# HKUST-Aerial-Robotics/A-LOAM

Hardware: AMD Instinct MI355X
Metric: HDL-64 scans/sec (whole node) (higher is better)
Workload: dtype f32 features / f64 solve

## Files before the change

a-loam_amd/csrc/aloam_capi.hip:

```cpp
#include <algorithm>
#include <cstdio>
#include <cstdlib>
#include <cstring>

#include "capi_internal.hpp"
#include "information_device.hpp"

namespace aloam {

hipEvent_t prof_event(aloam_ctx* c) {
  if (!c->prof_free.empty()) { hipEvent_t e = c->prof_free.back(); c->prof_free.pop_back(); return e; }
  Event e;
  (void)hipEventCreate(&e.h);
  c->prof_events.push_back(std::move(e));
  return c->prof_events.back();
}

int stage_ints(aloam_ctx* c, const int* src, int n, int* dst) {
  const int ns = c->h_nin_slot;
  c->h_nin_slot = (ns + 1) % kNinSlots;
  int* slot = c->h_nin.get() + (size_t)ns * c->B;
  if (c->nin_used[ns]) HIP_TRY(c, hipEventSynchronize(c->nin_done[ns]));
  std::memcpy(slot, src, sizeof(int) * n);
  HIP_TRY(c, hipMemcpyAsync(dst, slot, sizeof(int) * n, hipMemcpyHostToDevice, c->stream));
// ... 112 lines not shown
  { int cus = 0; if (hipDeviceGetAttribute(&cus, hipDeviceAttributeMultiprocessorCount, cfg->device) == hipSuccess && cus > 0) c->gather_blocks = 8 * cus; }
  if (reg) {
    c->slab = c->npad + 16;
    if ((rc = dmalloc(c, c->d_slabs, B * R * (size_t)c->slab))) return rc;
    if ((rc = dmalloc(c, c->d_front_lb, B * NB * (size_t)kFrontSlots))) return rc;
    if ((rc = dmalloc(c, c->d_front_ticket, B))) return rc;
    if ((rc = dmalloc(c, c->d_ringstart, B * (R + 1)))) return rc;
    if ((rc = dmalloc(c, c->d_curv, B * cap))) return rc;
    if ((rc = dmalloc(c, c->d_label, B * cap))) return rc;
    if ((rc = dmalloc(c, c->d_lookback, B * 4 * R))) return rc;
    if ((rc = dmalloc(c, c->d_ring_ticket, B))) return rc;
  }
  if (reg || odo) {
    if ((rc = dmalloc(c, c->d_sharp, B * R * kSharpPerRing))) return rc;
    if ((rc = dmalloc(c, c->d_flat, B * R * kFlatPerRing))) return rc;
  }
  for (int k = 0; k < 2; ++k) {
    if (!(odo || (k == 0 && reg) || (k == 1 && map))) continue;
    if ((rc = dmalloc(c, c->d_less_sharp[k], B * R * kLessSharpPerRing))) return rc;
    if ((rc = dmalloc(c, c->d_less_flat[k], B * cap))) return rc;
  }
  if (odo) {
    for (int p = 0; p < 2; ++p) for (int k = 0; k < 2; ++k) {
      const size_t per = k == 0 ? R * kLessSharpPerRing : cap;
      if ((rc = dmalloc(c, c->d_grid_sorted3[p][k], B * per))) return rc;
      if ((rc = dmalloc(c, c->d_grid_sorted2[p][k], B * per))) return rc;
      if ((rc = dmalloc(c, c->d_grid_start3[p][k], B * (c->grid_H[k] + 1)))) return rc;
      if ((rc = dmalloc(c, c->d_grid_start2[p][k], B * (c->grid_H[k] + 1)))) return rc;
      if ((rc = dmalloc(c, c->d_grid_sorted3c[p][k], B * per))) return rc;
      if ((rc = dmalloc(c, c->d_grid_start3c[p][k], B * (c->grid_H[k] + 1)))) return rc;
      if ((rc = dmalloc(c, c->d_grid_flags[p][k], B * 4))) return rc;
      if ((rc = dmalloc(c, c->d_grid_walk[p][k], B * 2 * (R + 8)))) return rc;
    }
    if (c->grid_overlap) {
      HIP_TRY(c, hipStreamCreateWithFlags(&c->grid_stream.h, hipStreamNonBlocking));
      HIP_TRY(c, hipEventCreateWithFlags(&c->grid_fork.h, hipEventDisableTiming));
      HIP_TRY(c, hipEventCreateWithFlags(&c->grids_done.h, hipEventDisableTiming));
    }
    if ((rc = dmalloc(c, c->d_edges, B * R * kSharpPerRing))) return rc;
    if ((rc = dmalloc(c, c->d_planes, B * R * kFlatPerRing))) return rc;
    if ((rc = dmalloc(c, c->d_sel_sharp, B * R * kSharpPerRing))) return rc;
    if ((rc = dmalloc(c, c->d_sel_flat, B * R * kFlatPerRing))) return rc;
    if ((rc = prepare_build_grids(c->grid_H[1]))) { c->err = "k_build_grids: dynamic LDS size rejected"; return ALOAM_E_HIP; }
  }
  std::vector<OdomState> init(B);
  std::memset(init.data(), 0, sizeof(OdomState) * B);
  for (size_t b = 0; b < B; ++b) { init[b].para_q[3] = 1.0; init[b].q_w[3] = 1.0; }
  HIP_TRY(c, hipMemcpyAsync(c->d_state.get(), init.data(), sizeof(OdomState) * B, hipMemcpyHostToDevice, c->stream));
  HIP_TRY(c, hipStreamSynchronize(c->stream));
  return ALOAM_OK;
}

void aloam_destroy(aloam_ctx* c) {
  DeviceScope device_scope(c);
  if (!c) return;
  if (c->stream) (void)hipStreamSynchronize(c->stream);
  if (c->copy_stream) (void)hipStreamSynchronize(c->copy_stream);
  if (c->grid_stream) (void)hipStreamSynchronize(c->grid_stream);
  prof_resolve(c);
  delete c;
}

const char* aloam_last_error(const aloam_ctx* c) { return c ? c->err.c_str() : "null context"; }
void* aloam_stream(aloam_ctx* c) { return c ? (void*)c->stream : nullptr; }

int aloam_synchronize(aloam_ctx* c) {
  DeviceScope device_scope(c);
// ... 162 lines not shown
```

a-loam_amd/csrc/aloam_device.hpp:

```cpp
#pragma once
#include <hip/hip_runtime.h>
#include <stdint.h>
#include "aloam_atan.hpp"

namespace aloam {

constexpr int kFrontSlots = 128 + 8;
constexpr int kBlockPts = 1024;
constexpr int kMaxRings = 128;
constexpr int kSectors = 6;
constexpr int kSharpPerSector = 2;
constexpr int kLessSharpPerSector = 20;
constexpr int kFlatPerSector = 4;
constexpr int kSharpPerRing = kSectors * kSharpPerSector;
constexpr int kLessSharpPerRing = kSectors * kLessSharpPerSector;
constexpr int kFlatPerRing = kSectors * kFlatPerSector;
constexpr int kNnTile = 1024;

enum ErrBits { kErrEmpty = 1, kErrRingCap = 2, kErrPointCap = 4, kErrInternal = 8 };

struct alignas(16) SeqMeta {
  int n_in;
  int first_kept, last_kept;
  int half_idx;
// ... 31 lines not shown
  int pt_stride;
  int B, cap, R, NB;
  int ring_from_field;
  float min_range;
  SeqMeta* meta;
  float4* slabs;
  int slab;
  unsigned long long* front_lb;
  int* front_ticket;
  int* ringstart;
  float4* cloud;
  float* curv;
  int8_t* label;
  unsigned long long* lookback;
  unsigned epoch;
  int* ring_ticket;
  int store_debug;
  float4* sharp;
  float4* less_sharp[2];
  float4* flat;
  float4* less_flat[2];
  const int* active;
};

constexpr int kRangeRowTables = 6;
struct RangeArgs {
  const int* n_cols;
  const float2* az_xy;
  const float* row_tab;
  int rows, n_az, row_major;
  float range_scale;
};

struct OdomArgs {
  int B, cap, R;
  SeqMeta* meta;
  OdomState* state;
  const float4* sharp;
  const float4* flat;
  const float4* less_sharp[2];
  const float4* less_flat[2];
  const int* active;
  float4* grid_sorted3[2][2];
  float4* grid_sorted2[2][2];
  int* grid_start3[2][2];
  int* grid_start2[2][2];
  float4* grid_sorted3c[2][2];
  int* grid_start3c[2][2];
  int* grid_flags[2][2];
  int* grid_walk[2][2];
  int grid_H_corner, grid_H_surf;
  float4* sel_sharp;
  float4* sel_flat;
  EdgeRec* edges;
  PlaneRec* planes;
  int outer;
  int last_outer;
  int lm_max_iterations;
  int distortion;
};

template <typename T>
__device__ __forceinline__ T* row_of(T* const (&buf)[2], int k, int b, long long per) { return (k ? buf[1] : buf[0]) + b * per; }
__device__ __forceinline__ const float4* corner_last(const OdomArgs& a, int b, int parity) { return row_of(a.less_sharp, parity ^ 1, b, (long long)a.R * kLessSharpPerRing); }
__device__ __forceinline__ const float4* surf_last(const OdomArgs& a, int b, int parity) { return row_of(a.less_flat, parity ^ 1, b, (long long)a.cap); }

struct GridView {
  int H;
  float4 *sorted3, *sorted2, *sorted3c;
  int *start3, *start2, *start3c, *flags, *walk;
};
template <typename T>
__device__ __forceinline__ T* grid_ptr(T* const (&buf)[2][2], int set, int which) {
  return set ? (which ? buf[1][1] : buf[1][0]) : (which ? buf[0][1] : buf[0][0]);
}
__device__ __forceinline__ GridView grid_view(const OdomArgs& a, int b, int which, int set) {
  GridView g;
  g.H = which == 0 ? a.grid_H_corner : a.grid_H_surf;
  const long long per = which == 0 ? (long long)a.R * kLessSharpPerRing : (long long)a.cap;
  g.sorted3 = grid_ptr(a.grid_sorted3, set, which) + b * per;
  g.sorted2 = grid_ptr(a.grid_sorted2, set, which) + b * per;
  g.start3 = grid_ptr(a.grid_start3, set, which) + (long long)b * (g.H + 1);
  g.start2 = grid_ptr(a.grid_start2, set, which) + (long long)b * (g.H + 1);
  g.sorted3c = grid_ptr(a.grid_sorted3c, set, which) + b * per;
// ... 185 lines not shown
```

a-loam_amd/csrc/capi_internal.hpp:

```cpp
#pragma once
#include <hip/hip_runtime.h>

#include <cstdio>
#include <memory>
#include <string>
#include <utility>
#include <vector>

#include "../../include/aloam_mi355x.h"
#include "aloam_device.hpp"
#include "atlas_kernels.hpp"
#include "checkpoint_kernels.hpp"
#include "export_kernels.hpp"
#include "mapping_kernels.hpp"
#include "odometry_kernels.hpp"
#include "places_kernels.hpp"
#include "posegraph_kernels.hpp"
#include "registration_kernels.hpp"
#include "relocalize_kernels.hpp"

using namespace aloam;

namespace aloam {
enum KernelId { K_FIND_ENDS = 0, K_FRONT, K_RING_STARTS, K_DENSE_CLOUD, K_RING_FEATURES, K_BUILD_GRIDS, K_TRANSFORM, K_ASSOC_CORNER,
// ... 71 lines not shown
  aloam_config cfg{};
  int stages = ALOAM_STAGE_ALL;
  int B = 0, cap = 0, R = 0, NB = 0, npad = 0;
  int max_points = 0;
  std::string err;
  DevBuf<char> d_in[2]; size_t d_in_bytes[2] = {0, 0};
  int in_slot = 0;
  bool in_used[2] = {false, false};
  DevBuf<int> d_nin;
  PinnedBuf<int> h_nin; int h_nin_slot = 0;
  bool nin_used[kNinSlots] = {};
  std::vector<SeqHost> seq;
  bool all_active = true, any_frozen = false, any_attached = false;
  bool reg_pending = false;
  const int* reg_mask = nullptr;
  DevBuf<int> d_mask_reg, d_mask_odo, d_mask_map, d_reset_ids;
  DevBuf<SeqMeta> d_meta;
  DevBuf<float4> d_slabs; int slab = 0;
  DevBuf<unsigned long long> d_front_lb; DevBuf<int> d_front_ticket;
  bool dense_valid = true;
  DevBuf<int> d_ringstart;
  DevBuf<float4> d_cloud; DevBuf<float> d_curv; DevBuf<int8_t> d_label;
  DevBuf<unsigned long long> d_lookback; unsigned reg_epoch = 0;
  DevBuf<int> d_ring_ticket;
  bool debug_arrays = false;
  DevBuf<float4> d_sharp, d_flat;
  DevBuf<float4> d_less_sharp[2], d_less_flat[2];
  DevBuf<OdomState> d_state;
  DevBuf<float4> d_grid_sorted3[2][2], d_grid_sorted2[2][2];
  DevBuf<int> d_grid_start3[2][2], d_grid_start2[2][2];
  DevBuf<float4> d_grid_sorted3c[2][2];
  DevBuf<int> d_grid_start3c[2][2];
  DevBuf<int> d_grid_flags[2][2], d_grid_walk[2][2];
  int grid_H[2] = {4096, 16384};
  bool grid_overlap = false;
  DevBuf<EdgeRec> d_edges; DevBuf<PlaneRec> d_planes;
  DevBuf<float4> d_sel_sharp, d_sel_flat;
  bool map_on = false;
  long long map_err_reported = 0;
  float map_line_res = 0.4f, map_plane_res = 0.8f;
  int map_levels = 0, map_stack_tile_bound = 0, map_nsegs_max = 0;
  MapPool map;
  int map_pool_limit = 1 << 26;
  int map_growths = 0;
  long long map_steps = 0;
  int nin_max = 0;
  int inject_max = 0;
  PinnedBuf<volatile int> h_map_report;
  int* d_map_report_host = nullptr;
  DevBuf<int> d_map_report, d_map_live;
  DevBuf<MapSeq> d_mapseq; DevBuf<CubeDesc> d_cubes; DevBuf<int> d_maptab;
  DevBuf<MapGridSig> d_grid_sig;
  DevBuf<float4> d_stack[2], d_stack_world[2]; DevBuf<int> d_stack_cube[2];
  DevBuf<int> d_addcnt, d_cursor, d_compact_flag;
  DevBuf<MapEdgeRec> d_medges; DevBuf<MapNormRec> d_mnorms; DevBuf<float4> d_registered, d_knn;
  DevBuf<int> d_vox_lists;
  DevBuf<int> d_rec_tiles; int rec_tiles_corner = 0, rec_tiles_per_seq = 0;
  DevBuf<VoxSeg> d_segs; DevBuf<int> d_vox_counters, d_bbox;
  DevBuf<int> d_exp_cnt, d_exp_chunk; DevBuf<long long> d_exp_off;
  DevBuf<int> d_exp_pref[2];
  int exp_last_segs = 0;
  int gather_blocks = 2048;
  DevBuf<float4> d_exp_tmp; long long exp_tmp_cap = 0;
  DevBuf<long long> d_exp_tmp_off;
  DevBuf<int> d_ck_seqs, d_ck_info, d_ck_units, d_ck_chunk, d_ck_pref; DevBuf<long long> d_ck_uoff;
  PinnedBuf<char> h_ck; char* d_ck_host = nullptr;
// ... 183 lines not shown
```

a-loam_amd/csrc/capi_odometry.hip:

```cpp
#include <algorithm>
#include <cstring>

#include "capi_internal.hpp"

namespace {

RegArgs reg_args(aloam_ctx* c, const void* d_scans, long long seq_stride, int pt_stride) {
  RegArgs a{};
  a.in = (const char*)d_scans; a.seq_stride = seq_stride; a.pt_stride = pt_stride;
  a.B = c->B; a.cap = c->cap; a.R = c->R; a.NB = c->NB;
  a.ring_from_field = c->cfg.ring_from_field; a.min_range = c->cfg.min_range;
  a.meta = c->d_meta.get(); a.slabs = c->d_slabs.get(); a.slab = c->slab; a.front_lb = c->d_front_lb.get(); a.front_ticket = c->d_front_ticket.get();
  a.ringstart = c->d_ringstart.get(); a.cloud = c->d_cloud.get(); a.curv = c->d_curv.get(); a.label = c->d_label.get();
  a.lookback = c->d_lookback.get(); a.epoch = c->reg_epoch; a.store_debug = c->debug_arrays ? 1 : 0; a.ring_ticket = c->d_ring_ticket.get();
  a.sharp = c->d_sharp.get(); a.flat = c->d_flat.get();
  for (int k = 0; k < 2; ++k) { a.less_sharp[k] = c->d_less_sharp[k].get(); a.less_flat[k] = c->d_less_flat[k].get(); }
  a.active = c->reg_mask;
  return a;
}

}

namespace aloam {

OdomArgs odom_args(aloam_ctx* c) {
  OdomArgs a{};
  a.B = c->B; a.cap = c->cap; a.R = c->R;
  a.meta = c->d_meta.get(); a.state = c->d_state.get();
  a.sharp = c->d_sharp.get(); a.flat = c->d_flat.get();
  for (int k = 0; k < 2; ++k) { a.less_sharp[k] = c->d_less_sharp[k].get(); a.less_flat[k] = c->d_less_flat[k].get(); }
  for (int p = 0; p < 2; ++p) for (int k = 0; k < 2; ++k) {
    a.grid_sorted3[p][k] = c->d_grid_sorted3[p][k].get(); a.grid_sorted2[p][k] = c->d_grid_sorted2[p][k].get(); a.grid_start3[p][k] = c->d_grid_start3[p][k].get();
    a.grid_sorted3c[p][k] = c->d_grid_sorted3c[p][k].get(); a.grid_start3c[p][k] = c->d_grid_start3c[p][k].get();
    a.grid_start2[p][k] = c->d_grid_start2[p][k].get();
    a.grid_flags[p][k] = c->d_grid_flags[p][k].get(); a.grid_walk[p][k] = c->d_grid_walk[p][k].get();
  }
  a.grid_H_corner = c->grid_H[0]; a.grid_H_surf = c->grid_H[1];
  a.edges = c->d_edges.get(); a.planes = c->d_planes.get();
  a.sel_sharp = c->d_sel_sharp.get(); a.sel_flat = c->d_sel_flat.get();
  a.lm_max_iterations = c->cfg.lm_max_iterations;
  a.distortion = c->cfg.distortion != 0;
  return a;
}

}

namespace {

int check_batch(aloam_ctx* c, const int* n_in, int stride_bytes) {
  if (const int rc = require_stage(c, ALOAM_STAGE_REGISTRATION)) return rc;
  if (stride_bytes < 12 || (stride_bytes & 3)) { c->err = "stride_bytes must be 12 (x, y, z only) or >= 16, and a multiple of 4"; return ALOAM_E_ARG; }
  if (stride_bytes == 12 && c->cfg.ring_from_field) { c->err = "ring_from_field needs the 4th float of every record: stride_bytes >= 16"; return ALOAM_E_ARG; }
  for (int b = 0; b < c->B; ++b) {
    if (n_in[b] < 0) { c->err = "negative point count"; return ALOAM_E_ARG; }
    if (n_in[b] > c->max_points) { c->err = "scan exceeds max_points"; return ALOAM_E_CAPACITY; }
  }
  return ALOAM_OK;
}

}

namespace aloam {

int register_launch(aloam_ctx* c, const void* d_scans, long long seq_stride, const int* n_in, int stride_bytes, int slot, bool debug_arrays, const int* n_cols) {
  int rc = ALOAM_OK;
  if (!c->all_active && (rc = ensure_dense(c))) return rc;
  c->nin_max = 0;
  for (int b = 0; b < c->B; ++b) if (takes_part(c, b)) c->nin_max = std::max(c->nin_max, n_in[b]);
  if ((rc = stage_ints(c, n_cols ? n_cols : n_in, c->B, c->d_nin.get()))) return rc;
  if (n_cols) c->range_cols.assign(n_cols, n_cols + c->B); else c->range_cols.clear();
// ... 143 lines not shown
  const int rc = stage_and_register(c, h_scans, seq_stride_bytes, n_in, stride_bytes, false);
  if (rc) return rc;
  return aloam_odometry_step(c);
}

int aloam_input_consumed(aloam_ctx* c) {
  DeviceScope device_scope(c);
  if (!c) return ALOAM_E_ARG;
  for (int s = 0; s < 2; ++s) if (c->in_used[s]) HIP_TRY(c, hipEventSynchronize(c->in_consumed[s]));
  return ALOAM_OK;
}

int aloam_odometry_step(aloam_ctx* c) {
  DeviceScope device_scope(c);
  if (!c) return ALOAM_E_ARG;
  if (const int rc = require_stage(c, ALOAM_STAGE_ODOMETRY)) return rc;
  if (!c->have_features) { c->err = "aloam_odometry_step before any features were registered / set"; return ALOAM_E_STATE; }
  StageMask m;
  if (const int rc = stage_mask(c, c->d_mask_odo, [](const SeqHost& s) { return s.inited ? (int)kSeqSolve : 0; },
                                [](const aloam_ctx* x, const StageMask& k) { return k.all_solve || (!k.any_solve && x->all_active); }, &m)) return rc;
  const int* mask = m.dev;
  const bool any_solve = m.any_solve;
  const bool overlap = c->grid_overlap;
  bool build_last = !overlap;
  if (overlap) for (int b = 0; b < c->B; ++b) build_last |= (m.bits[b] & kSeqSolve) && !c->seq[b].grid_built;
  hipError_t join_err = hipSuccess;
  const int cus = c->gather_blocks / 8;
  auto launch_all = [&]() {
    OdomArgs a = odom_args(c);
    a.active = mask;
    if (overlap) {
      hipError_t e = hipEventRecord(c->grid_fork, c->stream);
      if (e == hipSuccess) e = hipStreamWaitEvent(c->grid_stream, c->grid_fork, 0);
      { ProfScope p(c, K_BUILD_GRIDS, c->grid_stream); launch_build_grids(a, true, cus, c->grid_stream); }
      if (e == hipSuccess) e = hipEventRecord(c->grids_done, c->grid_stream);
      join_err = e;
    }
    if (any_solve && build_last) {
      if (overlap) launch_build_grids(a, false, cus, c->stream);
      else { ProfScope p(c, K_BUILD_GRIDS); launch_build_grids(a, false, cus, c->stream); }
    }
    for (int outer = 0; any_solve && outer < c->cfg.outer_iterations; ++outer) {
      a.outer = outer;
      a.last_outer = outer == c->cfg.outer_iterations - 1;
      { ProfScope p(c, K_TRANSFORM); launch_transform_queries(a, c->stream); }
      { ProfScope p(c, K_ASSOC_CORNER); launch_associate(a, false, c->stream); }
      { ProfScope p(c, K_ASSOC_PLANE); launch_associate(a, true, c->stream); }
      { ProfScope p(c, K_SOLVE); launch_solve(a, c->stream); }
    }
    if (overlap && join_err == hipSuccess) join_err = hipStreamWaitEvent(c->stream, c->grids_done, 0);
    { ProfScope p(c, K_ADVANCE); launch_advance(a, c->stream); }
  };
  if (!any_solve) {
    launch_all();
  } else if (c->use_graph && !c->prof_on && !c->debug_sync) {
    GraphExec& ge = c->odom_graph[mask ? 1 : 0];
    if (!ge) {
      hipGraph_t g = nullptr;
      hipError_t e = hipStreamBeginCapture(c->stream, hipStreamCaptureModeThreadLocal);
      if (e == hipSuccess) {
        launch_all();
        e = hipStreamEndCapture(c->stream, &g);
        if (e == hipSuccess) e = hipGraphInstantiate(&ge.h, g, nullptr, nullptr, 0);
        if (g) (void)hipGraphDestroy(g);
      }
      if (e != hipSuccess) {
        (void)hipGetLastError();
        ge.reset();
        c->use_graph = false;
      }
    }
    if (ge) HIP_TRY(c, hipGraphLaunch(ge, c->stream));
    else launch_all();
// ... 214 lines not shown
```

a-loam_amd/csrc/odometry_kernels.hip:

```cpp
#include "aloam_device.hpp"
#include "aloam_trig.hpp"
#include "lm_device.hpp"
#include "odometry_solve_device.hpp"
#include "odometry_kernels.hpp"

namespace aloam {

#define ALOAM_PHASE(name) asm volatile("; ##PHASE " name)
#ifdef ALOAM_PHASE_CLOCK
__device__ unsigned long long g_phase_clock_odo[2][32];
#define ALOAM_BG_CLOCK(slot) do { if (threadIdx.x == 0 && blockIdx.x == 1) { atomicAdd(&g_phase_clock_odo[0][slot], (unsigned long long)__builtin_readcyclecounter()); atomicAdd(&g_phase_clock_odo[1][slot], 1ull); } } while (0)
#else
#define ALOAM_BG_CLOCK(slot) do { } while (0)
#endif
#ifdef ALOAM_ASSOC_STATS
__device__ unsigned long long g_assoc_stats[2][32];
#define ALOAM_STAT(cls, i, v) do { if ((threadIdx.x & 63) == 0) atomicAdd(&g_assoc_stats[cls][i], (unsigned long long)(v)); } while (0)
#else
#define ALOAM_STAT(cls, i, v) do { } while (0)
#endif

__device__ __forceinline__ float4 transform_to_start(const float4& p, const OdomState& st) {
  double q[4] = {st.para_q[0], st.para_q[1], st.para_q[2], st.para_q[3]};
  if (q[3] < 0.0) { q[0] = -q[0]; q[1] = -q[1]; q[2] = -q[2]; q[3] = -q[3]; }
// ... 25 lines not shown
    const int i = base + tid;
    const int key = i < n ? (int)pts[i].w : -1;
    const int prev = __shfl_up(key, 1, 64), next = __shfl_down(key, 1, 64);
    if (key >= 0 && key < S) {
      if (lane == 0 || prev != key) atomicMin(&s_first[key], i);
      if (lane == 63 || next != key) atomicMax(&s_last[key], i);
    }
  }
  __syncthreads();
  if (tid == 0) {
    int run = n;
    for (int k = S - 1; k >= 0; --k) { run = min(run, s_first[k]); s_first[k] = run; walk[k] = run; }
    run = -1;
    for (int k = 0; k < S; ++k) { run = max(run, s_last[k]); s_last[k] = run; walk[S + k] = run; }
    bool nearly = true;
    for (int k = 3; k < S; ++k) nearly = nearly && s_last[k - 3] < s_first[k];
    s_flag[1] = nearly ? 1 : 2;
  }
  __syncthreads();
}
__host__ __device__ __forceinline__ bool fused_takes(int n, int H) { return n <= kFusedMaxN && H <= kFusedMaxH; }

template <bool NEXT>
struct BuildSrc {
  int n, set;
  const float4* pts;
  __device__ __forceinline__ BuildSrc(const OdomArgs& a, const SeqMeta& m, int b, int which) {
    set = NEXT ? m.parity : m.parity ^ 1;
    n = which == 0 ? (NEXT ? m.n_less_sharp : m.n_corner_last) : (NEXT ? m.n_less_flat : m.n_surf_last);
    pts = which == 0 ? row_of(a.less_sharp, set, b, (long long)a.R * kLessSharpPerRing) : row_of(a.less_flat, set, b, (long long)a.cap);
  }
};

template <bool NEXT>
__device__ __forceinline__ void build_grids_fused(const OdomArgs& a, int b, int which) {
  constexpr int U = 4;
  const int tid = threadIdx.x, lane = tid & 63, wave = tid >> 6;
  if (seq_idle(a.active, b, NEXT ? kSeqActive : kSeqSolve)) return;
  const SeqMeta m = a.meta[b];
  const BuildSrc<NEXT> src(a, m, b, which);
  const int n = src.n;
  const float4* pts = src.pts;
  const GridView g = grid_view(a, b, which, src.set);
  const int H = g.H;
  if (!fused_takes(n, H)) return;
  extern __shared__ __attribute__((aligned(16))) int lds[];
  unsigned* tab = reinterpret_cast<unsigned*>(lds);
  int* s_part = lds + 3 * (H / 2);
  int* s_flag = s_part + 48;
  int* s_walk = s_flag + 8;
  int* const starts[3] = {g.start3, g.start3c, g.start2};
  if (n == 0) {
    for (int t = 0; t < 3; ++t) for (int h = tid; h <= H; h += 1024) starts[t][h] = 0;
    if (tid < 3) g.flags[tid] = 0;
    return;
  }
  ALOAM_BG_CLOCK(0);
  for (int w = tid; w < 3 * (H / 2); w += 1024) tab[w] = 0u;
  if (tid < 2) s_flag[tid] = 0;
  __syncthreads();
  ALOAM_BG_CLOCK(1);
  const float inv0 = 1.0f / cell3_of(which), inv1 = 1.0f / (cell3_of(which) * kCell3CoarseFactor), inv2 = 1.0f / kCell2;
  const unsigned hm = (unsigned)(H - 1);
  auto buckets = [&](const float4& p, int key, unsigned* h) {
    h[0] = hash3((int)floorf(p.x * inv0), (int)floorf(p.y * inv0), (int)floorf(p.z * inv0)) & hm;
    h[1] = hash3((int)floorf(p.x * inv1), (int)floorf(p.y * inv1), (int)floorf(p.z * inv1)) & hm;
    h[2] = hash3((int)floorf(p.x * inv2), (int)floorf(p.y * inv2), key) & hm;
  };
  auto fetch = [&](int base, float4* p) {
#pragma unroll
    for (int u = 0; u < U; ++u) { const int i = base + u * 1024 + tid; p[u] = pts[i < n ? i : n - 1]; }
  };
  {
    int bad = 0, unsorted = 0;
    for (int base = 0; base < n; base += U * 1024) {
      float4 p[U];
      float pw[U];
      fetch(base, p);
// ... 47 lines not shown
    }
  }
  __syncthreads();
  ALOAM_BG_CLOCK(4);
  for (int base = 0; base < n; base += U * 1024) {
    float4 p[U];
    fetch(base, p);
#pragma unroll
    for (int u = 0; u < U; ++u) {
      const int i = base + u * 1024 + tid;
      if (i >= n) continue;
      const int key = (int)p[u].w;
      unsigned h[3];
      buckets(p[u], key, h);
      unsigned pos[3];
#pragma unroll
      for (int t = 0; t < 3; ++t) {
        const unsigned sh = (h[t] & 1u) * 16;
        pos[t] = (atomicAdd(&tab[t * (H / 2) + (h[t] >> 1)], 1u << sh) >> sh) & 0xffffu;
      }
      const float4 e = make_float4(p[u].x, p[u].y, p[u].z, __uint_as_float((unsigned)i | ((unsigned)(key + 1) << 20)));
      g.sorted3[pos[0]] = e;
      g.sorted3c[pos[1]] = e;
      g.sorted2[pos[2]] = e;
    }
  }
  ALOAM_BG_CLOCK(5);
#ifdef ALOAM_PHASE_CLOCK
  __syncthreads();
  ALOAM_BG_CLOCK(6);
#endif
}

__global__ __launch_bounds__(1024) void k_build_grids_fused(OdomArgs a) { build_grids_fused<false>(a, blockIdx.y, blockIdx.x); }
__global__ __launch_bounds__(1024) void k_build_grids_fused_next(OdomArgs a) {
  const int G = gridDim.x;
  for (int r = 0, i = blockIdx.x; i < 2 * a.B; ++r, i += G) {
    build_grids_fused<true>(a, i >> 1, (i ^ r) & 1);
    __syncthreads();
  }
}

constexpr int kBgWaves = 4;
constexpr int kBgUnroll = 4;
template <bool NEXT>
__device__ __forceinline__ void build_grids(const OdomArgs& a) {
  constexpr int U = kBgUnroll;
  const int b = blockIdx.y, which = blockIdx.x / 3, tid = threadIdx.x;
  const int pass_lo = blockIdx.x % 3, pass_hi = pass_lo + 1;
  if (seq_idle(a.active, b, NEXT ? kSeqActive : kSeqSolve)) return;
  const SeqMeta m = a.meta[b];
  const BuildSrc<NEXT> src(a, m, b, which);
  const int n = src.n;
  const float4* pts = src.pts;
  const GridView g = grid_view(a, b, which, src.set);
  if (fused_takes(n, g.H)) return;
  extern __shared__ __attribute__((aligned(16))) int lds[];
  int* cnt = lds;
  int* part = lds + g.H;
  int* s_flag = part + 1024;
  if (tid < 2) s_flag[tid] = n >= (1 << 20) && tid == 0 ? 1 : 0;
  if (n == 0) {
    for (int pass = pass_lo; pass < pass_hi; ++pass) { int* st = pass == 0 ? g.start3 : pass == 1 ? g.start3c : g.start2; for (int h = tid; h <= g.H; h += 1024) st[h] = 0; }
    if (tid < 3 && pass_lo == 0) g.flags[tid] = 0;
    return;
  }
  auto fetch = [&](int base, float4* p) {
#pragma unroll
    for (int u = 0; u < U; ++u) { const int i = base + u * 1024 + tid; p[u] = pts[i < n ? i : n - 1]; }
  };
  for (int pass = pass_lo; pass < pass_hi; ++pass) {
    const bool g3 = pass < 2;
    const float cell = pass == 0 ? cell3_of(which) : pass == 1 ? cell3_of(which) * kCell3CoarseFactor : kCell2;
    const float inv = 1.0f / cell;
    int* start = pass == 0 ? g.start3 : pass == 1 ? g.start3c : g.start2;
    float4* sorted = pass == 0 ? g.sorted3 : pass == 1 ? g.sorted3c : g.sorted2;
    __syncthreads();
    for (int h = tid; h < g.H; h += 1024) cnt[h] = 0;
    __syncthreads();
    float4 p[U], pn[U];
    float pw[U], pwn[U];
    fetch(0, p);
    if (pass == 0) {
#pragma unroll
      for (int u = 0; u < U; ++u) { const int i = u * 1024 + tid; pw[u] = pts[i < n ? (i > 0 ? i - 1 : 0) : n - 1].w; }
    }
    int bad = 0, unsorted = 0;
    for (int base = 0; base < n; base += U * 1024) {
      if (base + U * 1024 < n) {
// ... 21 lines not shown
    if (pass == 0) {
      if (bad) atomicOr(&s_flag[0], 1);
      if (unsorted) atomicOr(&s_flag[1], 1);
    }
    __syncthreads();
    if (pass == 0 && tid < 3) g.flags[tid] = tid == 2 ? 0 : (tid == 1 ? 2 * s_flag[1] : s_flag[0]);
    const int per = g.H / 1024;
    int local = 0;
    for (int k = 0; k < per; ++k) local += cnt[tid * per + k];
    int total;
    int run = block_exclusive_scan<int, 1024>(local, part, &total);
    for (int k = 0; k < per; ++k) { const int c = cnt[tid * per + k]; cnt[tid * per + k] = run; start[tid * per + k] = run; run += c; }
    if (tid == 1023) start[g.H] = run;
    __syncthreads();
    fetch(0, p);
    for (int base = 0; base < n; base += U * 1024) {
      if (base + U * 1024 < n) fetch(base + U * 1024, pn);
#pragma unroll
      for (int u = 0; u < U; ++u) {
        const int i = base + u * 1024 + tid;
        if (i >= n) continue;
        const int key = (int)p[u].w;
        const int ix = (int)floorf(p[u].x * inv), iy = (int)floorf(p[u].y * inv);
        const int iz = g3 ? (int)floorf(p[u].z * inv) : key;
        const int pos = atomicAdd(&cnt[hash3(ix, iy, iz) & (g.H - 1)], 1);
        sorted[pos] = make_float4(p[u].x, p[u].y, p[u].z, __uint_as_float((unsigned)i | ((unsigned)(key + 1) << 20)));
      }
#pragma unroll
      for (int u = 0; u < U; ++u) p[u] = pn[u];
    }
  }
}

__global__ __launch_bounds__(1024, kBgWaves) void k_build_grids(OdomArgs a) { build_grids<false>(a); }
__global__ __launch_bounds__(1024, kBgWaves) void k_build_grids_next(OdomArgs a) { build_grids<true>(a); }

__device__ __forceinline__ float walk_dist(const float4& p, const float4& sel) {
  return (p.x - sel.x) * (p.x - sel.x) + (p.y - sel.y) * (p.y - sel.y) + (p.z - sel.z) * (p.z - sel.z);
}

__device__ __forceinline__ unsigned long long wave_min_u64(unsigned long long v) {
  return wave_min_packed(v);
}

__device__ __forceinline__ void ring2d(int r, int t, int* dx, int* dy) {
  const int w = 2 * r + 1;
  if (t < w) { *dx = -r + t; *dy = -r; }
  else if (t < 2 * w) { *dx = -r + (t - w); *dy = r; }
  else { const int u = t - 2 * w, side = u / (w - 2); *dy = -r + 1 + u % (w - 2); *dx = side ? r : -r; }
}
__device__ __forceinline__ void shell3d(int r, int c, int* dx, int* dy, int* dz) {
  const int w = 2 * r + 1, nface = w * w;
  if (c < 2 * nface) { const int f = c / nface, q = c % nface; *dz = f ? r : -r; *dy = q / w - r; *dx = q % w - r; }
  else { const int q = c - 2 * nface; *dz = -r + 1 + q / (8 * r); ring2d(r, q % (8 * r), dx, dy); }
}

template <int kSweep> struct Kept { float4 p[kSweep]; bool a[kSweep]; bool ok; };

template <int kSweep, class F>
__device__ __forceinline__ void wave_sweep(const float4* __restrict__ sorted, int s0, int cnt, int lane, int* row, F&& f, Kept<kSweep>* keep = nullptr) {
  const int incl = wave_scan_i32<false>(cnt);
  const int total = __builtin_amdgcn_readlane(incl, 63);
  const int excl = incl - cnt;
  int carry = 0;
  for (int base = 0; base < total; base += kSweep * 64) {
    const int slot = excl - base;
    const int rows = total - base > (kSweep - 1) * 64 ? kSweep : (total - base + 63) >> 6;
#pragma unroll
// ... 769 lines not shown
    st.lm_iterations[o] = iterations;
    st.lm_successful[o] = successful;
    st.initial_cost[o] = initial_cost;
    st.final_cost[o] = cost;
    st.termination[o] = termination;
    if (a.last_outer) {
      const double qw[4] = {st.q_w[0], st.q_w[1], st.q_w[2], st.q_w[3]};
      double rt[3];
      quat_rotate(qw, t[0], t[1], t[2], rt);
      st.t_w[0] += rt[0]; st.t_w[1] += rt[1]; st.t_w[2] += rt[2];
      st.q_w[0] = qw[3] * q[0] + qw[0] * q[3] + qw[1] * q[2] - qw[2] * q[1];
      st.q_w[1] = qw[3] * q[1] + qw[1] * q[3] + qw[2] * q[0] - qw[0] * q[2];
      st.q_w[2] = qw[3] * q[2] + qw[2] * q[3] + qw[0] * q[1] - qw[1] * q[0];
      st.q_w[3] = qw[3] * q[3] - qw[0] * q[0] - qw[1] * q[1] - qw[2] * q[2];
    }
  }
}

__global__ void k_advance(SeqMeta* meta, OdomState* state, const int* active, int B) {
  const int b = blockIdx.x * blockDim.x + threadIdx.x;
  if (b >= B || seq_idle(active, b)) return;
  SeqMeta& m = meta[b];
  m.n_corner_last = m.n_less_sharp; m.n_surf_last = m.n_less_flat; m.parity ^= 1;
  state[b].inited = 1;
}
__global__ void k_set_inited(OdomState* state, int B, int inited) {
  const int b = blockIdx.x * blockDim.x + threadIdx.x;
  if (b < B) state[b].inited = inited;
}
void launch_set_inited(OdomState* state, int B, int inited, hipStream_t s) { hipLaunchKernelGGL(k_set_inited, dim3((B + 63) / 64), dim3(64), 0, s, state, B, inited); }
void launch_advance(const OdomArgs& a, hipStream_t s) { hipLaunchKernelGGL(k_advance, dim3((a.B + 63) / 64), dim3(64), 0, s, a.meta, a.state, a.active, a.B); }

size_t build_grids_lds_bytes(int H, int R) { return sizeof(int) * ((size_t)H + 1024 + 2 * (R + 8) + 4); }
static size_t build_grids_fused_lds_bytes(int H) { return sizeof(int) * (3 * (size_t)(H / 2) + 48 + 8 + 2 * kWalkKeys); }
int prepare_build_grids(int H_surf) {
  const int fused = (int)build_grids_fused_lds_bytes(kFusedMaxH), per_grid = (int)build_grids_lds_bytes(H_surf, kMaxRings);
  if (hipFuncSetAttribute((const void*)k_build_grids_fused, hipFuncAttributeMaxDynamicSharedMemorySize, fused) != hipSuccess) return -1;
  if (hipFuncSetAttribute((const void*)k_build_grids_fused_next, hipFuncAttributeMaxDynamicSharedMemorySize, fused) != hipSuccess) return -1;
  if (hipFuncSetAttribute((const void*)k_build_grids, hipFuncAttributeMaxDynamicSharedMemorySize, per_grid) != hipSuccess) return -1;
  return hipFuncSetAttribute((const void*)k_build_grids_next, hipFuncAttributeMaxDynamicSharedMemorySize, per_grid) == hipSuccess ? 0 : -1;
}
void launch_build_grids(const OdomArgs& a, bool next, int cus, hipStream_t s) {
  const int hc = a.grid_H_corner <= kFusedMaxH ? a.grid_H_corner : 0, hs = a.grid_H_surf <= kFusedMaxH ? a.grid_H_surf : 0;
  const size_t fused = build_grids_fused_lds_bytes(hc > hs ? hc : hs), per_grid = build_grids_lds_bytes(a.grid_H_surf, a.R);
  if (next) {
    const int wgs = cus / 2 >= 2 ? (cus / 2) & ~1 : 2;
    if (hc || hs) hipLaunchKernelGGL(k_build_grids_fused_next, dim3(2 * a.B < wgs ? 2 * a.B : wgs), dim3(1024), fused, s, a);
    hipLaunchKernelGGL(k_build_grids_next, dim3(6, a.B), dim3(1024), per_grid, s, a);
  } else {
    if (hc || hs) hipLaunchKernelGGL(k_build_grids_fused, dim3(2, a.B), dim3(1024), fused, s, a);
    hipLaunchKernelGGL(k_build_grids, dim3(6, a.B), dim3(1024), per_grid, s, a);
  }
}
void launch_transform_queries(const OdomArgs& a, hipStream_t s) {
  const dim3 grid((a.R * (kSharpPerRing + kFlatPerRing) + 255) / 256, a.B);
  if (a.distortion) hipLaunchKernelGGL(k_transform_queries<true>, grid, dim3(256), 0, s, a);
  else hipLaunchKernelGGL(k_transform_queries<false>, grid, dim3(256), 0, s, a);
}
void launch_associate(const OdomArgs& a, bool plane, hipStream_t s) {
  const int by = (a.B + 7) / 8 * 8;
  const int qcap = plane ? a.R * kFlatPerRing : a.R * kSharpPerRing;
  const bool wide = a.R > 64;
  const dim3 grid((unsigned)(qcap / 2 * by)), block(64), gridf((unsigned)a.B), blockf(256);
  const dim3 gridn((unsigned)((qcap / 2 + kPairsPerWave - 1) / kPairsPerWave), (unsigned)a.B);
  if (wide) {
    if (plane) { hipLaunchKernelGGL((k_associate_pair<true, true>), grid, block, 0, s, a); hipLaunchKernelGGL((k_associate_nearly<true, true>), gridn, block, 0, s, a); hipLaunchKernelGGL((k_associate_flagged<true, true>), gridf, blockf, 0, s, a); }
    else { hipLaunchKernelGGL((k_associate_pair<false, true>), grid, block, 0, s, a); hipLaunchKernelGGL((k_associate_nearly<false, true>), gridn, block, 0, s, a); hipLaunchKernelGGL((k_associate_flagged<false, true>), gridf, blockf, 0, s, a); }
  } else {
    if (plane) { hipLaunchKernelGGL((k_associate_pair<true, false>), grid, block, 0, s, a); hipLaunchKernelGGL((k_associate_nearly<true, false>), gridn, block, 0, s, a); hipLaunchKernelGGL((k_associate_flagged<true, false>), gridf, blockf, 0, s, a); }
    else { hipLaunchKernelGGL((k_associate_pair<false, false>), grid, block, 0, s, a); hipLaunchKernelGGL((k_associate_nearly<false, false>), gridn, block, 0, s, a); hipLaunchKernelGGL((k_associate_flagged<false, false>), gridf, blockf, 0, s, a); }
  }
}
void launch_solve(const OdomArgs& a, hipStream_t s) {
  if (a.distortion) hipLaunchKernelGGL(k_solve<true>, dim3(a.B), dim3(kSolveThreads), 0, s, a);
  else hipLaunchKernelGGL(k_solve<false>, dim3(a.B), dim3(kSolveThreads), 0, s, a);
}
}

#ifdef ALOAM_PHASE_CLOCK
extern "C" int aloam_debug_phase_clock_odo(unsigned long long* out) { return (int)hipMemcpyFromSymbol(out, HIP_SYMBOL(aloam::g_phase_clock_odo), sizeof(unsigned long long) * 64); }
#endif
#ifdef ALOAM_ASSOC_STATS
extern "C" int aloam_debug_assoc_stats(unsigned long long* out) { return (int)hipMemcpyFromSymbol(out, HIP_SYMBOL(aloam::g_assoc_stats), sizeof(unsigned long long) * 64); }
#endif
// ... 1 lines not shown
```

a-loam_amd/csrc/odometry_kernels.hpp:

```cpp
#pragma once
#include "aloam_device.hpp"

struct aloam_pose_information;

namespace aloam {
size_t build_grids_lds_bytes(int H, int R);
int prepare_build_grids(int H_surf);
void launch_build_grids(const OdomArgs& a, bool next, int cus, hipStream_t s);
void launch_transform_queries(const OdomArgs& a, hipStream_t s);
void launch_associate(const OdomArgs& a, bool plane, hipStream_t s);
void launch_solve(const OdomArgs& a, hipStream_t s);
void launch_advance(const OdomArgs& a, hipStream_t s);
void launch_pose_information_odom(const OdomArgs& a, const int* list, int n, aloam_pose_information* dst, hipStream_t s);
void launch_set_inited(OdomState* state, int B, int inited, hipStream_t s);
}
```

Measured before the change: 134,700.

## Build non-fused grids from a device work list with persistent workgroups

Fused grid builds that decline a cloud now append its three pass items to a device work list. The per-grid kernel then runs as a persistent grid sized to resident capacity and pulls items from that list with an atomic counter, replacing a 6xB launch where most blocks exited early. It also adds register caps and a kernarg reload trick to cut register pressure, plus an env knob to split the corner and surface fused launches. Risks include atomic contention, correctness of the list reset by the last block, and spills under the forced register limits.

```diff
diff --git a/a-loam_amd/csrc/aloam_capi.hip b/a-loam_amd/csrc/aloam_capi.hip
--- a/a-loam_amd/csrc/aloam_capi.hip
+++ b/a-loam_amd/csrc/aloam_capi.hip
@@ -168,7 +168,16 @@
       if ((rc = dmalloc(c, c->d_grid_flags[p][k], B * 4))) return rc;
       if ((rc = dmalloc(c, c->d_grid_walk[p][k], B * 2 * (R + 8)))) return rc;
     }
+    if ((rc = dmalloc(c, c->d_grid_list, 2 * grid_list_ints(c->B)))) return rc;
+    HIP_TRY(c, hipMemsetAsync(c->d_grid_list.get(), 0, sizeof(int) * 2 * grid_list_ints(c->B), c->stream));
     if (c->grid_overlap) {
+      const int cus = c->gather_blocks / 8;
+      c->grid_wgs[0] = cus / 2; c->grid_wgs[1] = 0;
+      if (const char* e = std::getenv("ALOAM_GRID_BUILD_WGS")) {
+        int gc = 0, gs = 0;
+        const int got = std::sscanf(e, "%d,%d", &gc, &gs);
+        if (got >= 1 && gc > 0 && gc <= 4096 && gs >= 0 && gs <= 4096) { c->grid_wgs[0] = gc; c->grid_wgs[1] = got == 2 ? gs : 0; }
+      }
       HIP_TRY(c, hipStreamCreateWithFlags(&c->grid_stream.h, hipStreamNonBlocking));
       HIP_TRY(c, hipEventCreateWithFlags(&c->grid_fork.h, hipEventDisableTiming));
       HIP_TRY(c, hipEventCreateWithFlags(&c->grids_done.h, hipEventDisableTiming));
diff --git a/a-loam_amd/csrc/aloam_device.hpp b/a-loam_amd/csrc/aloam_device.hpp
--- a/a-loam_amd/csrc/aloam_device.hpp
+++ b/a-loam_amd/csrc/aloam_device.hpp
@@ -87,6 +87,9 @@
   float range_scale;
 };
 
+constexpr int kGridListHead = 4;
+__host__ __device__ __forceinline__ size_t grid_list_ints(int B) { return (kGridListHead + 6 * (size_t)B + 31) & ~(size_t)31; }
+
 struct OdomArgs {
   int B, cap, R;
   SeqMeta* meta;
@@ -105,6 +108,7 @@
   int* grid_flags[2][2];
   int* grid_walk[2][2];
   int grid_H_corner, grid_H_surf;
+  int* grid_list;
   float4* sel_sharp;
   float4* sel_flat;
   EdgeRec* edges;
diff --git a/a-loam_amd/csrc/capi_internal.hpp b/a-loam_amd/csrc/capi_internal.hpp
--- a/a-loam_amd/csrc/capi_internal.hpp
+++ b/a-loam_amd/csrc/capi_internal.hpp
@@ -127,6 +127,8 @@
   DevBuf<float4> d_grid_sorted3c[2][2];
   DevBuf<int> d_grid_start3c[2][2];
   DevBuf<int> d_grid_flags[2][2], d_grid_walk[2][2];
+  DevBuf<int> d_grid_list;
+  int grid_wgs[2] = {0, 0};
   int grid_H[2] = {4096, 16384};
   bool grid_overlap = false;
   DevBuf<EdgeRec> d_edges; DevBuf<PlaneRec> d_planes;
diff --git a/a-loam_amd/csrc/capi_odometry.hip b/a-loam_amd/csrc/capi_odometry.hip
--- a/a-loam_amd/csrc/capi_odometry.hip
+++ b/a-loam_amd/csrc/capi_odometry.hip
@@ -36,6 +36,7 @@
     a.grid_flags[p][k] = c->d_grid_flags[p][k].get(); a.grid_walk[p][k] = c->d_grid_walk[p][k].get();
   }
   a.grid_H_corner = c->grid_H[0]; a.grid_H_surf = c->grid_H[1];
+  a.grid_list = c->d_grid_list.get();
   a.edges = c->d_edges.get(); a.planes = c->d_planes.get();
   a.sel_sharp = c->d_sel_sharp.get(); a.sel_flat = c->d_sel_flat.get();
   a.lm_max_iterations = c->cfg.lm_max_iterations;
@@ -245,13 +246,13 @@
     if (overlap) {
       hipError_t e = hipEventRecord(c->grid_fork, c->stream);
       if (e == hipSuccess) e = hipStreamWaitEvent(c->grid_stream, c->grid_fork, 0);
-      { ProfScope p(c, K_BUILD_GRIDS, c->grid_stream); launch_build_grids(a, true, cus, c->grid_stream); }
+      { ProfScope p(c, K_BUILD_GRIDS, c->grid_stream); launch_build_grids(a, true, cus, c->grid_wgs[0], c->grid_wgs[1], c->grid_stream); }
       if (e == hipSuccess) e = hipEventRecord(c->grids_done, c->grid_stream);
       join_err = e;
     }
     if (any_solve && build_last) {
-      if (overlap) launch_build_grids(a, false, cus, c->stream);
-      else { ProfScope p(c, K_BUILD_GRIDS); launch_build_grids(a, false, cus, c->stream); }
+      if (overlap) launch_build_grids(a, false, cus, 0, 0, c->stream);
+      else { ProfScope p(c, K_BUILD_GRIDS); launch_build_grids(a, false, cus, 0, 0, c->stream); }
     }
     for (int outer = 0; any_solve && outer < c->cfg.outer_iterations; ++outer) {
       a.outer = outer;
diff --git a/a-loam_amd/csrc/odometry_kernels.hip b/a-loam_amd/csrc/odometry_kernels.hip
--- a/a-loam_amd/csrc/odometry_kernels.hip
+++ b/a-loam_amd/csrc/odometry_kernels.hip
@@ -81,10 +81,18 @@
   }
 };
 
+__device__ __forceinline__ const OdomArgs& kernarg_again(const OdomArgs&) {
+  unsigned long long p = (unsigned long long)__builtin_amdgcn_kernarg_segment_ptr();
+  asm volatile("" : "+s"(p));
+  return *(const OdomArgs*)(const __attribute__((address_space(4))) OdomArgs*)p;
+}
 template <bool NEXT>
-__device__ __forceinline__ void build_grids_fused(const OdomArgs& a, int b, int which) {
+__device__ __forceinline__ int* grid_list_of(const OdomArgs& a) { return a.grid_list + (NEXT ? grid_list_ints(a.B) : 0); }
+
+template <bool NEXT>
+__device__ __forceinline__ void build_grids_fused(const OdomArgs& a, int b, int which, int tid) {
   constexpr int U = 4;
-  const int tid = threadIdx.x, lane = tid & 63, wave = tid >> 6;
+  const int lane = tid & 63, wave = tid >> 6;
   if (seq_idle(a.active, b, NEXT ? kSeqActive : kSeqSolve)) return;
   const SeqMeta m = a.meta[b];
   const BuildSrc<NEXT> src(a, m, b, which);
@@ -92,7 +100,14 @@
   const float4* pts = src.pts;
   const GridView g = grid_view(a, b, which, src.set);
   const int H = g.H;
-  if (!fused_takes(n, H)) return;
+  if (!fused_takes(n, H)) {
+    if (tid == 0) {
+      int* list = grid_list_of<NEXT>(a);
+      const int at = atomicAdd(&list[0], 3);
+      for (int t = 0; t < 3; ++t) list[kGridListHead + at + t] = b * 6 + which * 3 + t;
+    }
+    return;
+  }
   extern __shared__ __attribute__((aligned(16))) int lds[];
   unsigned* tab = reinterpret_cast<unsigned*>(lds);
   int* s_part = lds + 3 * (H / 2);
@@ -206,11 +221,13 @@
 #endif
 }
 
-__global__ __launch_bounds__(1024) void k_build_grids_fused(OdomArgs a) { build_grids_fused<false>(a, blockIdx.y, blockIdx.x); }
-__global__ __launch_bounds__(1024) void k_build_grids_fused_next(OdomArgs a) {
-  const int G = gridDim.x;
-  for (int r = 0, i = blockIdx.x; i < 2 * a.B; ++r, i += G) {
-    build_grids_fused<true>(a, i >> 1, (i ^ r) & 1);
+__global__ __launch_bounds__(1024) void k_build_grids_fused(OdomArgs a) { build_grids_fused<false>(a, blockIdx.y, blockIdx.x, threadIdx.x); }
+__global__ __launch_bounds__(1024) __attribute__((amdgpu_num_sgpr(80), amdgpu_num_vgpr(20))) void k_build_grids_fused_next(OdomArgs a, int cls) {
+  const int G = gridDim.x, clouds = cls < 0 ? 2 * a.B : a.B;
+  for (int r = 0, i = blockIdx.x; i < clouds; ++r, i += G) {
+    int tid = threadIdx.x;
+    asm volatile("" : "+v"(tid));
+    build_grids_fused<true>(kernarg_again(a), cls < 0 ? i >> 1 : i, cls < 0 ? (i ^ r) & 1 : cls, tid);
     __syncthreads();
   }
 }
@@ -218,17 +235,14 @@
 constexpr int kBgWaves = 4;
 constexpr int kBgUnroll = 4;
 template <bool NEXT>
-__device__ __forceinline__ void build_grids(const OdomArgs& a) {
+__device__ __forceinline__ void build_grid(const OdomArgs& a, int b, int which, int pass_lo, int tid) {
   constexpr int U = kBgUnroll;
-  const int b = blockIdx.y, which = blockIdx.x / 3, tid = threadIdx.x;
-  const int pass_lo = blockIdx.x % 3, pass_hi = pass_lo + 1;
-  if (seq_idle(a.active, b, NEXT ? kSeqActive : kSeqSolve)) return;
+  const int pass_hi = pass_lo + 1;
   const SeqMeta m = a.meta[b];
   const BuildSrc<NEXT> src(a, m, b, which);
   const int n = src.n;
   const float4* pts = src.pts;
   const GridView g = grid_view(a, b, which, src.set);
-  if (fused_takes(n, g.H)) return;
   extern __shared__ __attribute__((aligned(16))) int lds[];
   int* cnt = lds;
   int* part = lds + g.H;
@@ -316,8 +330,33 @@
   }
 }
 
-__global__ __launch_bounds__(1024, kBgWaves) void k_build_grids(OdomArgs a) { build_grids<false>(a); }
-__global__ __launch_bounds__(1024, kBgWaves) void k_build_grids_next(OdomArgs a) { build_grids<true>(a); }
+template <bool NEXT>
+__device__ __forceinline__ void build_grids(const OdomArgs& a, int walk) {
+  int* list = grid_list_of<NEXT>(a);
+  const int count = walk ? list[0] : 1;
+  if (count == 0) return;
+  __shared__ int s_take;
+  for (;;) {
+    int e = blockIdx.y * 6 + blockIdx.x;
+    if (walk) {
+      if (threadIdx.x == 0) s_take = atomicAdd(&list[1], 1);
+      __syncthreads();
+      const int k = __builtin_amdgcn_readfirstlane(s_take);
+      if (k >= count) break;
+      e = list[kGridListHead + k];
+    } else if (seq_idle(a.active, blockIdx.y, NEXT ? kSeqActive : kSeqSolve)) {
+      return;
+    }
+    int tid = threadIdx.x;
+    asm volatile("" : "+v"(tid));
+    build_grid<NEXT>(kernarg_again(a), e / 6, e % 6 / 3, e % 3, tid);
+    if (!walk) return;
+    __syncthreads();
+  }
+  if (threadIdx.x == 0 && atomicAdd(&list[2], 1) == (int)gridDim.x - 1) list[0] = list[1] = list[2] = 0;
+}
+__global__ __launch_bounds__(1024, kBgWaves) __attribute__((amdgpu_num_sgpr(64))) void k_build_grids(OdomArgs a, int walk) { build_grids<false>(a, walk); }
+__global__ __launch_bounds__(1024, kBgWaves) __attribute__((amdgpu_num_sgpr(64))) void k_build_grids_next(OdomArgs a, int walk) { build_grids<true>(a, walk); }
 
 __device__ __forceinline__ float walk_dist(const float4& p, const float4& sel) {
   return (p.x - sel.x) * (p.x - sel.x) + (p.y - sel.y) * (p.y - sel.y) + (p.z - sel.z) * (p.z - sel.z);
@@ -1153,6 +1192,7 @@
 void launch_advance(const OdomArgs& a, hipStream_t s) { hipLaunchKernelGGL(k_advance, dim3((a.B + 63) / 64), dim3(64), 0, s, a.meta, a.state, a.active, a.B); }
 
 size_t build_grids_lds_bytes(int H, int R) { return sizeof(int) * ((size_t)H + 1024 + 2 * (R + 8) + 4); }
+constexpr size_t kLdsPerCu = 160 * 1024;
 static size_t build_grids_fused_lds_bytes(int H) { return sizeof(int) * (3 * (size_t)(H / 2) + 48 + 8 + 2 * kWalkKeys); }
 int prepare_build_grids(int H_surf) {
   const int fused = (int)build_grids_fused_lds_bytes(kFusedMaxH), per_grid = (int)build_grids_lds_bytes(H_surf, kMaxRings);
@@ -1161,16 +1201,29 @@
   if (hipFuncSetAttribute((const void*)k_build_grids, hipFuncAttributeMaxDynamicSharedMemorySize, per_grid) != hipSuccess) return -1;
   return hipFuncSetAttribute((const void*)k_build_grids_next, hipFuncAttributeMaxDynamicSharedMemorySize, per_grid) == hipSuccess ? 0 : -1;
 }
-void launch_build_grids(const OdomArgs& a, bool next, int cus, hipStream_t s) {
+void launch_build_grids(const OdomArgs& a, bool next, int cus, int wgs_corner, int wgs_surf, hipStream_t s) {
   const int hc = a.grid_H_corner <= kFusedMaxH ? a.grid_H_corner : 0, hs = a.grid_H_surf <= kFusedMaxH ? a.grid_H_surf : 0;
   const size_t fused = build_grids_fused_lds_bytes(hc > hs ? hc : hs), per_grid = build_grids_lds_bytes(a.grid_H_surf, a.R);
+  if (!hc && !hs) {
+    if (next) hipLaunchKernelGGL(k_build_grids_next, dim3(6, a.B), dim3(1024), per_grid, s, a, 0);
+    else hipLaunchKernelGGL(k_build_grids, dim3(6, a.B), dim3(1024), per_grid, s, a, 0);
+    return;
+  }
+  const int resident = cus * (2 * per_grid <= kLdsPerCu ? 2 : 1), walk = 6 * a.B < resident ? 6 * a.B : resident;
   if (next) {
-    const int wgs = cus / 2 >= 2 ? (cus / 2) & ~1 : 2;
-    if (hc || hs) hipLaunchKernelGGL(k_build_grids_fused_next, dim3(2 * a.B < wgs ? 2 * a.B : wgs), dim3(1024), fused, s, a);
-    hipLaunchKernelGGL(k_build_grids_next, dim3(6, a.B), dim3(1024), per_grid, s, a);
+    auto even = [](int w) { return w >= 2 ? w & ~1 : 2; };
+    if (wgs_surf > 0) {
+      const int gc = wgs_corner < a.B ? wgs_corner : a.B, gs = wgs_surf < a.B ? wgs_surf : a.B;
+      hipLaunchKernelGGL(k_build_grids_fused_next, dim3(gc > 0 ? gc : 1), dim3(1024), build_grids_fused_lds_bytes(hc), s, a, 0);
+      hipLaunchKernelGGL(k_build_grids_fused_next, dim3(gs), dim3(1024), build_grids_fused_lds_bytes(hs), s, a, 1);
+    } else {
+      const int wgs = even(wgs_corner);
+      hipLaunchKernelGGL(k_build_grids_fused_next, dim3(2 * a.B < wgs ? 2 * a.B : wgs), dim3(1024), fused, s, a, -1);
+    }
+    hipLaunchKernelGGL(k_build_grids_next, dim3(walk), dim3(1024), per_grid, s, a, 1);
   } else {
-    if (hc || hs) hipLaunchKernelGGL(k_build_grids_fused, dim3(2, a.B), dim3(1024), fused, s, a);
-    hipLaunchKernelGGL(k_build_grids, dim3(6, a.B), dim3(1024), per_grid, s, a);
+    hipLaunchKernelGGL(k_build_grids_fused, dim3(2, a.B), dim3(1024), fused, s, a);
+    hipLaunchKernelGGL(k_build_grids, dim3(walk), dim3(1024), per_grid, s, a, 1);
   }
 }
 void launch_transform_queries(const OdomArgs& a, hipStream_t s) {
diff --git a/a-loam_amd/csrc/odometry_kernels.hpp b/a-loam_amd/csrc/odometry_kernels.hpp
--- a/a-loam_amd/csrc/odometry_kernels.hpp
+++ b/a-loam_amd/csrc/odometry_kernels.hpp
@@ -6,7 +6,7 @@
 namespace aloam {
 size_t build_grids_lds_bytes(int H, int R);
 int prepare_build_grids(int H_surf);
-void launch_build_grids(const OdomArgs& a, bool next, int cus, hipStream_t s);
+void launch_build_grids(const OdomArgs& a, bool next, int cus, int wgs_corner, int wgs_surf, hipStream_t s);
 void launch_transform_queries(const OdomArgs& a, hipStream_t s);
 void launch_associate(const OdomArgs& a, bool plane, hipStream_t s);
 void launch_solve(const OdomArgs& a, hipStream_t s);
```

After: 134,300. About the same (-0.2%).
